# Python-for-HPC/ramba

Measured on NVIDIA H100. Metric: fused-elementwise GB/s (fp64 sin/cos/mul/add chain), higher is better.
Workload: dtype f64

## Files before the change

### ramba_b200/csrc/rb200_lean.cuh

```cuda
#pragma once
#include <cuda_runtime.h>
#include <stdint.h>

#include "rb200_vm.cuh"

namespace rb200 {

constexpr int LV = 8;

enum LeanKind { L_ACC = 0, L_REG = 1, L_SCAL = 2, L_STAGED = 3, L_DIRECT = 4, L_NONE = 7 };
enum LeanOp {
  LO_MOV = 0, LO_ADD, LO_SUB, LO_RSUB, LO_MUL, LO_DIV, LO_NEG, LO_ABS, LO_SQUARE, LO_MIN, LO_MAX,
  LO_MULADD, LO_MULSUB, LO_MULRSUB, LO_CVT, LO_RED, LO_CHAIN, LO_NUM
};

struct LInsn {
  unsigned char handler;
  unsigned char a_kind, b_kind, c_kind;
  unsigned char a_arg, b_arg, c_arg;
  unsigned char st_reg;
  unsigned char st_view;
  unsigned char red_op;
  unsigned char pad[2];
};

enum LeanChainOp { LC_ADD = 0, LC_SUB = 1, LC_RSUB = 2, LC_MUL = 3 };
struct LChainStep {
  unsigned char op, staged, pad[2];
};

struct LDirect {
  char* base;
  long long s0, s1, s2;
  int dtype;
  int pad;
};

template <class F> struct LAcc;
template <> struct LAcc<double> {
  static __device__ __forceinline__ double get(unsigned lo, unsigned hi) { return __hiloint2double((int)hi, (int)lo); }
  static __device__ __forceinline__ void put(double v, unsigned& lo, unsigned& hi) {
    lo = (unsigned)__double2loint(v);
    hi = (unsigned)__double2hiint(v);
  }
};
template <> struct LAcc<float> {
  static __device__ __forceinline__ float get(unsigned lo, unsigned) { return __uint_as_float(lo); }
  static __device__ __forceinline__ void put(float v, unsigned& lo, unsigned&) { lo = __float_as_uint(v); }
};

template <class F> __device__ __forceinline__ F lean_lds(unsigned addr);
template <> __device__ __forceinline__ double lean_lds<double>(unsigned addr) { return __longlong_as_double((long long)lds64(addr)); }
template <> __device__ __forceinline__ float lean_lds<float>(unsigned addr) { return __uint_as_float(lds32(addr)); }
template <class F> __device__ __forceinline__ void lean_sts(unsigned addr, F v);
template <> __device__ __forceinline__ void lean_sts<double>(unsigned addr, double v) { sts64(addr, (u64)__double_as_longlong(v)); }
template <> __device__ __forceinline__ void lean_sts<float>(unsigned addr, float v) {
  asm volatile("st.shared.u32 [%0], %1;" ::"r"(addr), "r"(__float_as_uint(v)) : "memory");
}

template <class F> struct LOther;
template <> struct LOther<double> { typedef float type; };
template <> struct LOther<float> { typedef double type; };

template <class F> __device__ __forceinline__ F l_add(F a, F b);
template <> __device__ __forceinline__ double l_add<double>(double a, double b) { return __dadd_rn(a, b); }
template <> __device__ __forceinline__ float l_add<float>(float a, float b) { return __fadd_rn(a, b); }
template <class F> __device__ __forceinline__ F l_sub(F a, F b);
template <> __device__ __forceinline__ double l_sub<double>(double a, double b) { return __dsub_rn(a, b); }
template <> __device__ __forceinline__ float l_sub<float>(float a, float b) { return __fsub_rn(a, b); }
template <class F> __device__ __forceinline__ F l_mul(F a, F b);
template <> __device__ __forceinline__ double l_mul<double>(double a, double b) { return __dmul_rn(a, b); }
template <> __device__ __forceinline__ float l_mul<float>(float a, float b) { return __fmul_rn(a, b); }
template <class F> __device__ __forceinline__ F l_div(F a, F b);
template <> __device__ __forceinline__ double l_div<double>(double a, double b) { return __ddiv_rn(a, b); }
template <> __device__ __forceinline__ float l_div<float>(float a, float b) { return __fdiv_rn(a, b); }

template <int LOP, class F, bool AACC, class CX> __device__ __forceinline__ void lean_exec(CX& cx, const LInsn& I) {
  F r[LV];
  if constexpr (LOP == LO_CVT) {
    typedef typename LOther<F>::type S;
    S s[LV];
    if constexpr (AACC) {
#pragma unroll
      for (int k = 0; k < LV; ++k) s[k] = LAcc<S>::get(cx.alo[k], cx.ahi[k]);
    } else {
      cx.template fetch<S>(I.a_kind, I.a_arg, s);
    }
#pragma unroll
    for (int k = 0; k < LV; ++k) r[k] = (F)s[k];
  } else {
    F a[LV];
    if constexpr (AACC) {
#pragma unroll
      for (int k = 0; k < LV; ++k) a[k] = LAcc<F>::get(cx.alo[k], cx.ahi[k]);
    } else {
      cx.template fetch<F>(I.a_kind, I.a_arg, a);
    }
    if constexpr (LOP == LO_MOV) {
#pragma unroll
      for (int k = 0; k < LV; ++k) r[k] = a[k];
    } else if constexpr (LOP == LO_CHAIN) {
#pragma unroll
      for (int k = 0; k < LV; ++k) r[k] = a[k];
#pragma unroll 1
      for (int s = 0; s < (int)I.c_arg; ++s) {
        F b[LV];
        const int cop = cx.template chain_fetch<F>((int)I.b_arg + s, b);
        if (cop == LC_ADD) {
#pragma unroll
          for (int k = 0; k < LV; ++k) r[k] = l_add<F>(r[k], b[k]);
        } else if (cop == LC_SUB) {
#pragma unroll
          for (int k = 0; k < LV; ++k) r[k] = l_sub<F>(r[k], b[k]);
        } else if (cop == LC_RSUB) {
#pragma unroll
          for (int k = 0; k < LV; ++k) r[k] = l_sub<F>(b[k], r[k]);
        } else {
#pragma unroll
          for (int k = 0; k < LV; ++k) r[k] = l_mul<F>(r[k], b[k]);
        }
      }
    } else if constexpr (LOP == LO_NEG) {
#pragma unroll
      for (int k = 0; k < LV; ++k) r[k] = -a[k];
    } else if constexpr (LOP == LO_ABS) {
#pragma unroll
      for (int k = 0; k < LV; ++k) r[k] = (F)fabs(a[k]);
    } else if constexpr (LOP == LO_SQUARE) {
#pragma unroll
      for (int k = 0; k < LV; ++k) r[k] = l_mul<F>(a[k], a[k]);
    } else if constexpr (LOP == LO_RED) {
      cx.template reduce<F>(I.b_arg, I.red_op, a);
      return;
    } else {
      F b[LV];
      cx.template fetch<F>(I.b_kind, I.b_arg, b);
      if constexpr (LOP == LO_ADD) {
#pragma unroll
        for (int k = 0; k < LV; ++k) r[k] = l_add<F>(a[k], b[k]);
      } else if constexpr (LOP == LO_SUB) {
#pragma unroll
        for (int k = 0; k < LV; ++k) r[k] = l_sub<F>(a[k], b[k]);
      } else if constexpr (LOP == LO_RSUB) {
#pragma unroll
        for (int k = 0; k < LV; ++k) r[k] = l_sub<F>(b[k], a[k]);
      } else if constexpr (LOP == LO_MUL) {
#pragma unroll
        for (int k = 0; k < LV; ++k) r[k] = l_mul<F>(a[k], b[k]);
      } else if constexpr (LOP == LO_DIV) {
#pragma unroll
        for (int k = 0; k < LV; ++k) r[k] = l_div<F>(a[k], b[k]);
      } else if constexpr (LOP == LO_MIN) {
#pragma unroll
        for (int k = 0; k < LV; ++k) r[k] = (b[k] < a[k]) ? b[k] : a[k];
      } else if constexpr (LOP == LO_MAX) {
#pragma unroll
        for (int k = 0; k < LV; ++k) r[k] = (b[k] > a[k]) ? b[k] : a[k];
      } else {
        F c[LV];
        cx.template fetch<F>(I.c_kind, I.c_arg, c);
#pragma unroll
        for (int k = 0; k < LV; ++k) {
          const F p = l_mul<F>(b[k], c[k]);
          r[k] = LOP == LO_MULADD ? l_add<F>(a[k], p) : LOP == LO_MULSUB ? l_sub<F>(a[k], p) : l_sub<F>(p, a[k]);
        }
      }
    }
  }
  if constexpr (LOP != LO_RED) {
#pragma unroll
    for (int k = 0; k < LV; ++k) LAcc<F>::put(r[k], cx.alo[k], cx.ahi[k]);
    if (I.st_reg != RB200_NOSTORE) cx.template store_reg<F>(I.st_reg, r);
    if (I.st_view != RB200_NOSTORE) cx.template store_view<F>(I.st_view, r);
  }
}

#define RB200_LEAN_CASE(LOP)                                             \
  case (LOP) * 4 + 0: lean_exec<LOP, double, false>(cx, I); break;       \
  case (LOP) * 4 + 1: lean_exec<LOP, double, true>(cx, I); break;        \
  case (LOP) * 4 + 2: lean_exec<LOP, float, false>(cx, I); break;        \
  case (LOP) * 4 + 3: lean_exec<LOP, float, true>(cx, I); break;

template <class CX> __device__ __forceinline__ void lean_dispatch(CX& cx, const LInsn& I) {
  switch (I.handler) {
    RB200_LEAN_CASE(LO_MOV)
    RB200_LEAN_CASE(LO_ADD)
    RB200_LEAN_CASE(LO_SUB)
    RB200_LEAN_CASE(LO_RSUB)
    RB200_LEAN_CASE(LO_MUL)
    RB200_LEAN_CASE(LO_DIV)
    RB200_LEAN_CASE(LO_NEG)
    RB200_LEAN_CASE(LO_ABS)
    RB200_LEAN_CASE(LO_SQUARE)
    RB200_LEAN_CASE(LO_MIN)
    RB200_LEAN_CASE(LO_MAX)
    RB200_LEAN_CASE(LO_MULADD)
    RB200_LEAN_CASE(LO_MULSUB)
    RB200_LEAN_CASE(LO_MULRSUB)
    RB200_LEAN_CASE(LO_CVT)
    RB200_LEAN_CASE(LO_RED)
    RB200_LEAN_CASE(LO_CHAIN)
    default: break;
  }
}

}
```

### ramba_b200/csrc/rb200_lean_plan.h

```cpp
#pragma once
#include <string.h>

#include "rb200_lean.cuh"

namespace rb200 {

static inline int lean_opcode(const rb200_fused_op* op, const rb200_insn& I) {
  switch (I.op) {
    case RB200_OP_MOV: return LO_MOV;
    case RB200_OP_ADD: return LO_ADD;
    case RB200_OP_SUB: return LO_SUB;
    case RB200_OP_MUL: return LO_MUL;
    case RB200_OP_DIV: return LO_DIV;
    case RB200_OP_NEG: return LO_NEG;
    case RB200_OP_ABS: return LO_ABS;
    case RB200_OP_SQUARE: return LO_SQUARE;
    case RB200_OP_MIN: return LO_MIN;
    case RB200_OP_MAX: return LO_MAX;
    case RB200_OP_MULADD: return LO_MULADD;
    case RB200_OP_MULSUB: return LO_MULSUB;
    case RB200_OP_MULRSUB: return LO_MULRSUB;
    case RB200_OP_RED: return LO_RED;
    case RB200_OP_POWI:
      if (I.b_kind == RB200_K_SCAL && (long long)op->scalars[I.b_idx] == 2) return LO_SQUARE;
      return -1;
    case RB200_OP_CVT: {
      const int src = (int)(I.imm & 0xff);
      if ((I.imm >> 8) != 0) return -1;
      if (!(src == RB200_T_F64 || src == RB200_T_F32) || src == (int)I.ctype) return -1;
      return LO_CVT;
    }
    default: return -1;
  }
}

static inline bool lean_eligible(const rb200_fused_op* op, bool allow_red) {
  if (op->n_insns < 1) return false;
  for (int i = 0; i < op->n_views; ++i)
    if (op->views[i].dtype != RB200_F32 && op->views[i].dtype != RB200_F64) return false;
  for (int i = 0; i < op->n_insns; ++i) {
    const rb200_insn& I = op->insns[i];
    if (I.ctype != RB200_T_F64 && I.ctype != RB200_T_F32) return false;
    if (I.mask_reg != RB200_NOSTORE) return false;
    const int lop = lean_opcode(op, I);
    if (lop < 0) return false;
    if (lop == LO_RED && (!allow_red || I.ctype != RB200_T_F64)) return false;
    const uint8_t kinds[3] = {I.a_kind, I.b_kind, I.c_kind};
    for (int q = 0; q < 3; ++q) {
      if (lop == LO_RED && q == 1) continue;
      if (kinds[q] == RB200_K_IOTA) return false;
    }
    if (I.a_kind == RB200_K_NONE) return false;
  }
  return true;
}

static inline void lean_translate(const rb200_fused_op* op, const int* view_kind, const int* view_arg, const int* store_arg, LInsn* out) {
  for (int i = 0; i < op->n_insns; ++i) {
    const rb200_insn& I = op->insns[i];
    LInsn L;
    memset(&L, 0, sizeof(L));
    int lop = lean_opcode(op, I);
    uint8_t kinds[3] = {I.a_kind, I.b_kind, I.c_kind};
    uint8_t idxs[3] = {I.a_idx, I.b_idx, I.c_idx};
    if (lop == LO_SQUARE || lop == LO_RED) kinds[1] = RB200_K_NONE;
    if ((lop == LO_ADD || lop == LO_MUL) && kinds[0] != RB200_K_ACC && kinds[1] == RB200_K_ACC) {
      kinds[1] = kinds[0]; idxs[1] = idxs[0];
      kinds[0] = RB200_K_ACC; idxs[0] = 0;
    } else if (lop == LO_SUB && kinds[0] != RB200_K_ACC && kinds[1] == RB200_K_ACC) {
      lop = LO_RSUB;
      kinds[1] = kinds[0]; idxs[1] = idxs[0];
      kinds[0] = RB200_K_ACC; idxs[0] = 0;
    }
    unsigned char lk[3], la[3];
    for (int q = 0; q < 3; ++q) {
      switch (kinds[q]) {
        case RB200_K_ACC: lk[q] = L_ACC; la[q] = 0; break;
        case RB200_K_REG: lk[q] = L_REG; la[q] = idxs[q]; break;
        case RB200_K_SCAL: lk[q] = L_SCAL; la[q] = idxs[q]; break;
        case RB200_K_VIEW: lk[q] = (unsigned char)view_kind[idxs[q]]; la[q] = (unsigned char)view_arg[idxs[q]]; break;
        default: lk[q] = L_NONE; la[q] = 0;
      }
    }
    L.a_kind = lk[0]; L.a_arg = la[0];
    L.b_kind = lk[1]; L.b_arg = la[1];
    L.c_kind = lk[2]; L.c_arg = la[2];
    if (lop == LO_RED) {
      L.b_arg = I.b_idx;
      L.red_op = (unsigned char)I.imm;
    }
    L.st_reg = I.st_reg;
    L.st_view = I.st_view == RB200_NOSTORE ? (unsigned char)RB200_NOSTORE : (unsigned char)store_arg[I.st_view];
    L.handler = (unsigned char)(lop * 4 + (I.ctype == RB200_T_F32 ? 2 : 0) + (L.a_kind == L_ACC ? 1 : 0));
    out[i] = L;
  }
}

static inline int lean_fuse_chains(LInsn* insns, int n, LChainStep* chain, int max_chain, int* n_chain_out) {
  int out = 0, nc = 0;
  int i = 0;
  auto chain_op = [](const LInsn& L) -> int {
    const int lop = L.handler >> 2;
    return lop == LO_ADD ? LC_ADD : lop == LO_SUB ? LC_SUB : lop == LO_RSUB ? LC_RSUB : lop == LO_MUL ? LC_MUL : -1;
  };
  while (i < n) {
    const LInsn first = insns[i];
    int j = i;
    if (chain_op(first) >= 0 && first.b_kind == L_STAGED) {
      const int cls = (first.handler >> 1) & 1;
      j = i + 1;
      while (j < n && insns[j - 1].st_reg == RB200_NOSTORE && insns[j - 1].st_view == RB200_NOSTORE && chain_op(insns[j]) >= 0 &&
             insns[j].b_kind == L_STAGED && insns[j].a_kind == L_ACC && ((insns[j].handler >> 1) & 1) == cls && nc + (j - i) + 1 <= max_chain && (j - i) < 200)
        ++j;
      if (j - i >= 2) {
        LInsn L = first;
        L.handler = (unsigned char)(LO_CHAIN * 4 + cls * 2 + (first.a_kind == L_ACC ? 1 : 0));
        L.b_kind = L_NONE;
        L.b_arg = (unsigned char)nc;
        L.c_arg = (unsigned char)(j - i);
        L.st_reg = insns[j - 1].st_reg;
        L.st_view = insns[j - 1].st_view;
        for (int q = i; q < j; ++q) {
          chain[nc].op = (unsigned char)chain_op(insns[q]);
          chain[nc].staged = insns[q].b_arg;
          ++nc;
        }
        insns[out++] = L;
        i = j;
        continue;
      }
    }
    insns[out++] = first;
    ++i;
  }
  *n_chain_out = nc;
  return out;
}

}
```

### ramba_b200/csrc/rb200_stream.cu

```cuda
#include <cuda_runtime.h>
#include <stdio.h>
#include <string.h>

#include <string>

#include "rb200_launch.h"
#include "rb200_lean.cuh"
#include "rb200_lean_plan.h"
#include "rb200_terms.h"
#include "rb200_mapred.h"
#include "rb200_stream.h"

namespace rb200 {

struct StreamCtx {
  const StreamParams& P;
  unsigned stage_s;
  unsigned reg_s;
  unsigned tid;
  bool staged_ok;
  long long row, e0;
  unsigned valid;
  unsigned alo[LV], ahi[LV];
  double racc[RB200_MAX_REDS];
// ... 74 lines not shown
  template <class F> __device__ __forceinline__ void reduce(int slot, int rop, const F (&a)[LV]) {
    if constexpr (sizeof(F) == 8) {
      if (P.mode == 1) {
#pragma unroll
        for (int k = 0; k < LV; ++k) cacc[k] = red_combine<double>(rop, cacc[k], a[k]);
        return;
      }
      double x[LV];
      const double ident = CT<double>::get(red_identity_bits(rop, RB200_T_F64));
#pragma unroll
      for (int k = 0; k < LV; ++k) x[k] = ((valid >> k) & 1u) ? (double)a[k] : ident;
#pragma unroll
      for (int w = LV / 2; w > 0; w >>= 1) {
#pragma unroll
        for (int k = 0; k < w; ++k) x[k] = red_combine<double>(rop, x[k], x[k + w]);
      }
#pragma unroll
      for (int s = 0; s < RB200_MAX_REDS; ++s)
        if (s == slot) racc[s] = red_combine<double>(rop, racc[s], x[0]);
    }
  }
};

__device__ __forceinline__ void stream_finish_reductions(const StreamParams& P, const double (&racc)[RB200_MAX_REDS]) {
  if (P.n_reds > 0) {
    __shared__ u64 wpart[RB200_MAX_REDS][kThreads / 32];
    __shared__ bool is_last;
    const int lane = threadIdx.x & 31, warp = threadIdx.x >> 5;
    for (int s = 0; s < P.n_reds; ++s) {
      const int op = P.reds[s].op;
      double mine = 0.0;
#pragma unroll
      for (int q = 0; q < RB200_MAX_REDS; ++q)
        if (q == s) mine = racc[q];
      u64 v = CT<double>::bits(mine);
#pragma unroll
      for (int o = 16; o > 0; o >>= 1) v = red_combine_bits(op, RB200_T_F64, v, __shfl_down_sync(0xffffffffu, v, o));
      if (lane == 0) wpart[s][warp] = v;
    }
    __syncthreads();
    if (threadIdx.x == 0) {
      for (int s = 0; s < P.n_reds; ++s) {
        const int op = P.reds[s].op;
        u64 v = wpart[s][0];
        for (int q = 1; q < kThreads / 32; ++q) v = red_combine_bits(op, RB200_T_F64, v, wpart[s][q]);
        P.red_partials[(long long)s * gridDim.x + blockIdx.x] = v;
      }
      __threadfence();
      const unsigned prev = atomicAdd(P.red_counter, 1u);
      is_last = (prev == gridDim.x - 1);
    }
    __syncthreads();
    if (is_last) {
      __threadfence();
      for (int s = 0; s < P.n_reds; ++s) {
        const int op = P.reds[s].op;
        u64 v = red_identity_bits(op, RB200_T_F64);
        for (unsigned b = threadIdx.x; b < gridDim.x; b += kThreads)
          v = red_combine_bits(op, RB200_T_F64, v, __ldcg(&P.red_partials[(long long)s * gridDim.x + b]));
#pragma unroll
        for (int o = 16; o > 0; o >>= 1) v = red_combine_bits(op, RB200_T_F64, v, __shfl_down_sync(0xffffffffu, v, o));
        __syncthreads();
        if (lane == 0) wpart[s][warp] = v;
        __syncthreads();
        if (threadIdx.x == 0) {
          v = wpart[s][0];
          for (int q = 1; q < kThreads / 32; ++q) v = red_combine_bits(op, RB200_T_F64, v, wpart[s][q]);
          const double vd = CT<double>::get(v);
          void* out = P.reds[s].out;
          if (P.reds[s].out_dtype == RB200_F64) {
            double* o = (double*)out;
            *o = red_combine<double>(op, *o, vd);
          } else {
            float* o = (float*)out;
            *o = (float)red_combine<double>(op, (double)*o, vd);
          }
        }
      }
      if (threadIdx.x == 0) *P.red_counter = 0u;
    }
  }
}

__global__ void __launch_bounds__(kThreads, 2) stream_kernel(const __grid_constant__ StreamParams P) {
  extern __shared__ __align__(128) unsigned char smem_raw[];
  const unsigned smem_s = (unsigned)__cvta_generic_to_shared(smem_raw);
  const unsigned tid = threadIdx.x;
  const unsigned ring_bytes = (unsigned)P.depth * P.stage_bytes;
  const unsigned regs_s = smem_s + ring_bytes;
  const unsigned mbar_s = regs_s + (unsigned)(P.n_regs + P.n_hoist) * (LV * kThreads * 8);
  if (P.n_staged > 0 && tid == 0) {
    for (int s = 0; s < P.depth; ++s) mbar_init(mbar_s + 8u * s, 1u);
    asm volatile("fence.mbarrier_init.release.cluster;" ::: "memory");
  }
  __syncthreads();

  StreamCtx cx(P);
  cx.tid = tid;
  cx.reg_s = regs_s + tid * 8u;
#pragma unroll
  for (int s = 0; s < RB200_MAX_REDS; ++s) cx.racc[s] = 0.0;
  for (int s = 0; s < P.n_reds; ++s) {
    const double ident = CT<double>::get(red_identity_bits(P.reds[s].op, RB200_T_F64));
#pragma unroll
    for (int q = 0; q < RB200_MAX_REDS; ++q)
      if (q == s) cx.racc[q] = ident;
  }

  long long n_it, base0, step_it;
  long long split = 0, col0 = 0, r0 = 0;
  if (P.mode == 0) {
    n_it = (P.n_tiles - (long long)blockIdx.x + gridDim.x - 1) / gridDim.x;
    base0 = (long long)blockIdx.x * kStreamTile;
    step_it = (long long)gridDim.x * kStreamTile;
    cx.row = 0;
  } else {
    split = blockIdx.x / (unsigned)P.n_chunks;
    const long long chunk = blockIdx.x - split * P.n_chunks;
    col0 = chunk * kStreamTile;
    r0 = split * P.rows_per_split;
    long long r1 = r0 + P.rows_per_split;
    if (r1 > P.R) r1 = P.R;
    n_it = r1 > r0 ? r1 - r0 : 0;
    base0 = r0 * P.C + col0;
    step_it = P.C;
    const double ident = CT<double>::get(red_identity_bits(P.reds[0].op, RB200_T_F64));
#pragma unroll
    for (int k = 0; k < LV; ++k) cx.cacc[k] = ident;
    cx.e0 = col0 + tid;
    cx.valid = (1u << LV) - 1u;
    cx.row = 0;
    cx.staged_ok = false;
    for (int h = 0; h < P.n_hoist; ++h) {
      if (P.hoist[h].is_f32_class) {
        float v[LV];
        cx.fetch_direct<float>(P.hoist[h].direct, v);
        cx.store_reg<float>(P.hoist[h].reg, v);
      } else {
        double v[LV];
        cx.fetch_direct<double>(P.hoist[h].direct, v);
        cx.store_reg<double>(P.hoist[h].reg, v);
      }
    }
  }

  auto tile_full = [&](long long it) -> bool { return P.mode == 1 || base0 + it * step_it + kStreamTile <= P.total; };
  auto issue = [&](long long it) {
    if (tid != 0) return;
    const unsigned slot = (unsigned)(it % P.depth);
    const unsigned bar = mbar_s + 8u * slot;
    const unsigned dst = smem_s + slot * P.stage_bytes;
    const long long eoff = base0 + it * step_it;
    unsigned bytes = 0;
    for (int j = 0; j < P.n_staged; ++j) bytes += (unsigned)(kStreamTile * P.staged[j].es);
    mbar_expect_tx(bar, bytes);
    for (int j = 0; j < P.n_staged; ++j)
      bulk_g2s(dst + P.staged[j].off, P.staged[j].base + eoff * P.staged[j].es, (unsigned)(kStreamTile * P.staged[j].es), bar);
  };

  if (P.n_staged > 0) {
    for (long long it = 0; it < P.depth - 1 && it < n_it; ++it)
      if (tile_full(it)) issue(it);
  }
  for (long long it = 0; it < n_it; ++it) {
    const bool full = tile_full(it);
    if (P.n_staged > 0) {
      __syncthreads();
      const long long nx = it + P.depth - 1;
      if (nx < n_it && tile_full(nx)) issue(nx);
      if (full) mbar_wait(mbar_s + 8u * (unsigned)(it % P.depth), (unsigned)((it / P.depth) & 1));
    }
    cx.staged_ok = full && P.n_staged > 0;
    cx.stage_s = smem_s + (unsigned)(it % (P.depth > 0 ? P.depth : 1)) * P.stage_bytes;
    if (P.mode == 0) {
      const long long e = base0 + it * step_it + tid;
      cx.e0 = e;
      unsigned valid = (1u << LV) - 1u;
      if (!full) {
        valid = 0;
#pragma unroll
        for (int k = 0; k < LV; ++k)
          if (e + (long long)k * kThreads < P.total) valid |= 1u << k;
      }
      cx.valid = valid;
    } else {
      cx.row = r0 + it;
    }
#pragma unroll 1
    for (int pc = 0; pc < P.n_insns; ++pc) {
      const LInsn I = P.insns[pc];
      lean_dispatch(cx, I);
    }
  }

  if (P.mode == 1) {
#pragma unroll
    for (int k = 0; k < LV; ++k) P.red_partials[split * P.C + col0 + tid + (long long)k * kThreads] = CT<double>::bits(cx.cacc[k]);
    return;
  }
  stream_finish_reductions(P, cx.racc);
}


template <int TV> struct STermCtx {
  unsigned stage_s, hoist_s, tid;
  bool staged_ok;
  long long row, e0;
  unsigned valid;
};

__device__ __forceinline__ void ip_add(double& a, double b) { asm("add.rn.f64 %0, %0, %1;" : "+d"(a) : "d"(b)); }
__device__ __forceinline__ void ip_sub(double& a, double b) { asm("sub.rn.f64 %0, %0, %1;" : "+d"(a) : "d"(b)); }
__device__ __forceinline__ void ip_rsub(double& a, double b) { asm("sub.rn.f64 %0, %1, %0;" : "+d"(a) : "d"(b)); }
__device__ __forceinline__ void ip_mul(double& a, double b) { asm("mul.rn.f64 %0, %0, %1;" : "+d"(a) : "d"(b)); }
__device__ __forceinline__ void ip_add(float& a, float b) { asm("add.rn.f32 %0, %0, %1;" : "+f"(a) : "f"(b)); }
__device__ __forceinline__ void ip_sub(float& a, float b) { asm("sub.rn.f32 %0, %0, %1;" : "+f"(a) : "f"(b)); }
__device__ __forceinline__ void ip_rsub(float& a, float b) { asm("sub.rn.f32 %0, %1, %0;" : "+f"(a) : "f"(b)); }
__device__ __forceinline__ void ip_mul(float& a, float b) { asm("mul.rn.f32 %0, %0, %1;" : "+f"(a) : "f"(b)); }

template <int TV, class F>
__device__ __forceinline__ void sterm_fetch(const StreamParams& P, const STermCtx<TV>& cx, const TermStep t, F (&x)[TV]) {
  int dview = t.xidx;
  if (t.xkind == X_STAGED) {
    const StreamStaged& sv = P.staged[t.xidx];
    if (cx.staged_ok) {
      if (sv.es == 4) {
        const unsigned addr = cx.stage_s + sv.off + cx.tid * 4u;
#pragma unroll
        for (int k = 0; k < TV; ++k) x[k] = (F)lean_lds<float>(addr + k * kThreads * 4);
      } else {
        const unsigned addr = cx.stage_s + sv.off + cx.tid * 8u;
#pragma unroll
        for (int k = 0; k < TV; ++k) x[k] = (F)lean_lds<double>(addr + k * kThreads * 8);
      }
      return;
    }
    dview = sv.dview;
  } else if (t.xkind == X_HOIST) {
    const unsigned base = cx.hoist_s + (unsigned)t.xidx * (TV * kThreads * 8);
    if (P.direct[P.thoist_direct[t.xidx]].dtype == RB200_F32) {
#pragma unroll
      for (int k = 0; k < TV; ++k) x[k] = (F)lean_lds<float>(base + cx.tid * 4u + k * kThreads * 4);
    } else {
#pragma unroll
      for (int k = 0; k < TV; ++k) x[k] = (F)lean_lds<double>(base + cx.tid * 8u + k * kThreads * 8);
    }
    return;
  }
  const LDirect& v = P.direct[dview];
  const long long off = cx.row * v.s1 + cx.e0 * v.s2;
  const long long step = (long long)kThreads * v.s2;
  if (v.dtype == RB200_F32) {
    const float* p = reinterpret_cast<const float*>(v.base) + off;
#pragma unroll
    for (int k = 0; k < TV; ++k, p += step) x[k] = ((cx.valid >> k) & 1u) ? (F)ldg<float>(p) : F(0);
  } else {
    const double* p = reinterpret_cast<const double*>(v.base) + off;
#pragma unroll
    for (int k = 0; k < TV; ++k, p += step) x[k] = ((cx.valid >> k) & 1u) ? (F)ldg<double>(p) : F(0);
  }
}

template <int TV, class F> __device__ __forceinline__ void sterm_store(const StreamParams& P, const STermCtx<TV>& cx, int dview, const F (&acc)[TV]) {
  const LDirect& v = P.direct[dview];
  const bool full = cx.valid == (TV == 32 ? 0xffffffffu : (1u << TV) - 1u);
  if (v.dtype == RB200_F32) {
    char* p = v.base + (cx.row * v.s1 + cx.e0 * v.s2) * 4;
    const long long step = (long long)kThreads * v.s2 * 4;
    if (full) {
#pragma unroll
      for (int k = 0; k < TV; ++k, p += step) stg<float>(reinterpret_cast<float*>(p), (float)acc[k]);
    } else {
#pragma unroll
      for (int k = 0; k < TV; ++k, p += step)
// ... 217 lines not shown
  __syncthreads();

  auto tile_full = [&](long long it) -> bool { return P.mode == 1 || base0 + it * step_it + TILE <= P.total; };
  auto issue = [&](long long it, int slot) {
    if (tid != 0) return;
    const unsigned bar = mbar_s + 8u * (unsigned)slot;
    const unsigned dst = smem_s + (unsigned)slot * P.stage_bytes;
    const long long eoff = base0 + it * step_it;
    mbar_expect_tx(bar, P.stage_bytes);
    for (int j = 0; j < P.n_staged; ++j)
      bulk_g2s(dst + P.staged[j].off, P.staged[j].base + eoff * P.staged[j].es, (unsigned)(TILE * P.staged[j].es), bar);
  };
  int islot = 0;
  if (P.n_staged > 0) {
    for (long long it = 0; it < P.depth - 1 && it < n_it; ++it) {
      if (tile_full(it)) issue(it, islot);
      islot = islot + 1 >= P.depth ? 0 : islot + 1;
    }
  }
  int slot = 0;
  unsigned par = 0;
  for (long long it = 0; it < n_it; ++it) {
    const bool full = tile_full(it);
    if (P.n_staged > 0) {
      __syncthreads();
      const long long nx = it + P.depth - 1;
      if (nx < n_it) {
        if (tile_full(nx)) issue(nx, islot);
        islot = islot + 1 >= P.depth ? 0 : islot + 1;
      }
      if (full) {
        mbar_wait(mbar_s + 8u * (unsigned)slot, (par >> slot) & 1u);
        par ^= 1u << slot;
      }
    }
    cx.staged_ok = full && P.n_staged > 0;
    cx.stage_s = smem_s + (unsigned)slot * P.stage_bytes;
    slot = slot + 1 >= P.depth ? 0 : slot + 1;
    if (P.mode == 0) {
      const long long e = base0 + it * step_it + tid;
      cx.e0 = e;
      unsigned valid = TV == 32 ? 0xffffffffu : (1u << TV) - 1u;
      if (!full) {
        valid = 0;
#pragma unroll
        for (int k = 0; k < TV; ++k)
          if (e + (long long)k * kThreads < P.total) valid |= 1u << k;
      }
      cx.valid = valid;
    } else {
      cx.row = r0 + it;
    }
    if (P.n32 > 0) {
      float a32[TV];
      sterm_steps<TV, float>(P, cx, 0, P.n32, a32, cacc, racc);
      if (P.n_terms > P.n32) {
        double a64[TV];
#pragma unroll
        for (int k = 0; k < TV; ++k) a64[k] = (double)a32[k];
        sterm_steps<TV, double>(P, cx, P.n32, P.n_terms, a64, cacc, racc);
      }
    } else {
      double a64[TV];
      sterm_steps<TV, double>(P, cx, 0, P.n_terms, a64, cacc, racc);
    }
  }

  if (P.mode == 1) {
#pragma unroll
    for (int k = 0; k < TV; ++k) P.red_partials[split * P.C + col0 + tid + (long long)k * kThreads] = CT<double>::bits(cacc[k]);
    return;
  }
  stream_finish_reductions(P, racc);
}


static bool stream_translate(const rb200_fused_op* op, StreamParams& P, bool column_mode, long long row_len) {
  bool rd[RB200_MAX_VIEWS] = {false};
  for (int i = 0; i < op->n_insns; ++i) {
    const rb200_insn& I = op->insns[i];
    const int lop = lean_opcode(op, I);
    if (I.a_kind == RB200_K_VIEW) rd[I.a_idx] = true;
    if (I.b_kind == RB200_K_VIEW && lop != LO_RED && lop != LO_SQUARE) rd[I.b_idx] = true;
    if (I.c_kind == RB200_K_VIEW) rd[I.c_idx] = true;
  }
  int view_kind[RB200_MAX_VIEWS], view_arg[RB200_MAX_VIEWS], store_arg[RB200_MAX_VIEWS];
  unsigned off = 0;
  for (int v = 0; v < op->n_views; ++v) {
    const rb200_view& vw = op->views[v];
    const int es = vw.dtype == RB200_F64 ? 8 : 4;
    LDirect& d = P.direct[P.n_direct];
    d.base = (char*)vw.base;
    d.s0 = 0;
    d.s1 = column_mode ? vw.stride[0] : 0;
    d.s2 = column_mode ? vw.stride[1] : vw.stride[0];
    d.dtype = vw.dtype;
    view_kind[v] = L_DIRECT;
    view_arg[v] = store_arg[v] = P.n_direct;
    const bool contiguous = d.s2 == 1 && (!column_mode || d.s1 == row_len);
    const bool aligned = (((uintptr_t)vw.base) & 15u) == 0 && (!column_mode || (row_len * es) % 16 == 0);
    if (rd[v] && contiguous && aligned && P.n_staged < kStreamMaxStaged) {
      StreamStaged& s = P.staged[P.n_staged];
      s.base = (const char*)vw.base;
      s.es = es;
      s.dview = P.n_direct;
      s.off = off;
      off += (unsigned)(kStreamTile * es);
      view_kind[v] = L_STAGED;
      view_arg[v] = P.n_staged;
      ++P.n_staged;
    }
    ++P.n_direct;
  }
  P.stage_bytes = off;
  P.n_insns = op->n_insns;
  P.n_regs = op->n_regs;
  lean_translate(op, view_kind, view_arg, store_arg, P.insns);
  for (int i = 0; i < op->n_scalars; ++i) P.scal[i] = op->scalars[i];
  return true;
}

static void stream_hoist_lean(StreamParams& P) {
    for (int dv = 0; dv < P.n_direct && P.n_hoist < kStreamMaxStaged; ++dv) {
      if (P.direct[dv].s1 != 0 || P.direct[dv].s2 != 1) continue;
      int cls = -1;
      bool same = true, used = false;
      for (int i = 0; i < P.n_insns; ++i) {
        const LInsn& L = P.insns[i];
        const int lop = L.handler >> 2;
        int fcls = (L.handler >> 1) & 1;
        if (lop == LO_CVT) fcls = 1 - fcls;
        const bool uses = (L.a_kind == L_DIRECT && L.a_arg == dv) || (L.b_kind == L_DIRECT && L.b_arg == dv) || (L.c_kind == L_DIRECT && L.c_arg == dv);
        if (!uses) continue;
        used = true;
        if (cls < 0) cls = fcls;
        else if (cls != fcls) same = false;
      }
      if (!used || !same) continue;
      const int reg = P.n_regs + P.n_hoist;
      if (reg >= 255) break;
      P.hoist[P.n_hoist].direct = dv;
      P.hoist[P.n_hoist].reg = reg;
      P.hoist[P.n_hoist].is_f32_class = cls;
      ++P.n_hoist;
      for (int i = 0; i < P.n_insns; ++i) {
        LInsn& L = P.insns[i];
        if (L.a_kind == L_DIRECT && L.a_arg == dv) { L.a_kind = L_REG; L.a_arg = (unsigned char)reg; }
        if (L.b_kind == L_DIRECT && L.b_arg == dv) { L.b_kind = L_REG; L.b_arg = (unsigned char)reg; }
        if (L.c_kind == L_DIRECT && L.c_arg == dv) { L.c_kind = L_REG; L.c_arg = (unsigned char)reg; }
      }
    }
  }

static void stream_layout(StreamParams& P) {
  unsigned off = 0;
  for (int j = 0; j < P.n_staged; ++j) {
    P.staged[j].off = off;
    off += (unsigned)(P.tv * kThreads * P.staged[j].es);
  }
  P.stage_bytes = off;
}

static size_t stream_smem(StreamParams& P) {
  const size_t tile = (size_t)P.tv * kThreads;
  const size_t regs = P.n_terms > 0 ? (size_t)P.n_thoist * tile * 8 : (size_t)(P.n_regs + P.n_hoist) * LV * kThreads * 8;
  const size_t budget = P.n_terms > 0 ? 70 * 1024 : 100 * 1024;
  if (regs + 1024 > budget) return 0;
  int depth = 0;
  if (P.n_staged > 0) {
    depth = (int)((budget - regs - 256) / P.stage_bytes);
    if (depth > 8) depth = 8;
    if (depth < 2) return 0;
  }
  P.depth = depth;
  return (size_t)depth * P.stage_bytes + regs + (size_t)(depth > 0 ? depth : 1) * 8 + 16;
}

bool plan_stream(const rb200_fused_op* op, int sms, int max_red_blocks, int n_split, bool use_terms, bool use_mapred, StreamPlan& T) {
  StreamParams& P = T.P;
  memset(&T, 0, sizeof(T));
  const bool column = op->n_axis_red_dims != 0;
  if (!column) {
    if (op->ndim != 1) return false;
    if (!lean_eligible(op, true)) return false;
    for (int s = 0; s < op->n_reds; ++s) {
      if (op->reds[s].ctype != RB200_T_F64) return false;
      if (op->reds[s].out_dtype != RB200_F64 && op->reds[s].out_dtype != RB200_F32) return false;
    }
    P.mode = 0;
    P.total = op->itershape[0];
  } else {
    if (op->ndim != 2 || op->n_axis_red_dims != 1 || op->n_reds != 1) return false;
    if (!lean_eligible(op, true)) return false;
    if (op->reds[0].ctype != RB200_T_F64) return false;
    const long long R = op->itershape[0], C = op->itershape[1];
    if (C % (LV * kThreads) != 0 || R < 2) return false;
    for (int i = 0; i < op->n_insns; ++i)
      if (op->insns[i].st_view != RB200_NOSTORE) return false;
    for (int v = 0; v < op->n_views; ++v) {
      const rb200_view& vw = op->views[v];
      if (vw.stride[1] != 1 || !(vw.stride[0] == C || vw.stride[0] == 0)) return false;
    }
    P.mode = 1;
    P.R = R;
    P.C = C;
    P.total = R * C;
  }
  P.tv = LV;
  stream_translate(op, P, column, P.C);
  TermBuild tb;
  tb.n_regs = P.n_regs;
  tb.direct = P.direct;
  tb.stream = true;
  tb.staged_fill = [](void*, int, int, TermStep*) -> bool { return true; };
  tb.ctx = nullptr;
  int out_view = -1;
  if (use_terms && build_terms(tb, P.insns, P.n_insns, P.terms, kMaxTerms, &P.n_terms, &P.n32, &out_view)) {
    auto src_of = [](void* ctx, const TermStep& t) -> MrSource {
      const StreamParams* Q = (const StreamParams*)ctx;
      MrSource r = {nullptr, 0, false};
      const LDirect* d = nullptr;
      if (t.xkind == X_STAGED) d = &Q->direct[Q->staged[t.xidx].dview];
      else if (t.xkind == X_DIRECT) d = &Q->direct[t.xidx];
      if (!d || d->s2 != 1) return r;
      if (Q->mode == 1 && !(d->s1 == Q->C || d->s1 == 0)) return r;
      r.base = d->base;
      r.f32 = d->dtype == RB200_F32;
      r.row_broadcast = Q->mode == 1 && d->s1 == 0;
      return r;
    };
    if (use_mapred && op->n_reds == 1 && mapred_try(P.mode, P.terms, P.n_terms, P.n32, P.scal, src_of, &P, &T.mr) == 0) {
      MrParams& M = T.mr;
      const int vec = M.src_f32 ? 4 : 2;
      bool ok = true;
      if (!column) {
        M.total = P.total;
        M.red.op = op->reds[0].op;
        M.red.ctype = op->reds[0].ctype;
        M.red.out = op->reds[0].out;
        M.red.out_dtype = op->reds[0].out_dtype;
        M.red_counter = (unsigned int*)op->red_scratch;
        M.red_partials = (u64*)((char*)op->red_scratch + 256);
        long long blocks = (P.total / (vec * 4) + kThreads - 1) / kThreads;
        long long cap = (long long)sms * 8;
        if (cap > max_red_blocks) cap = max_red_blocks;
        if (blocks > cap) blocks = cap;
        if (blocks < 1) blocks = 1;
        T.blocks = blocks;
      } else {
        const long long chunk = (long long)kThreads * vec;
        if (P.C % chunk != 0 || (P.C * (M.src_f32 ? 4 : 8)) % 16 != 0) ok = false;
        if (ok) {
          M.R = P.R;
          M.C = P.C;
          M.n_chunks = (int)(P.C / chunk);
          int eff = (int)(((long long)sms * 8) / M.n_chunks);
          if (n_split > 0 && eff > n_split) eff = n_split;
          if ((long long)eff > P.R) eff = (int)P.R;
          if (eff < 1) eff = 1;
          M.n_split = eff;
          M.rows_per_split = (P.R + eff - 1) / eff;
          M.red_partials = (u64*)op->red_scratch;
          T.eff = eff;
          T.blocks = (long long)eff * M.n_chunks;
        }
      }
      if (ok) {
        T.use_mr = true;
        T.smem = 0;
        return true;
      }
    }
    stream_layout(P);
    if (column) {
      for (int i = 0; i < P.n_terms; ++i) {
        TermStep& t = P.terms[i];
        if (t.xkind != X_DIRECT || P.direct[t.xidx].s1 != 0 || P.direct[t.xidx].s2 != 1) continue;
        int h = -1;
        for (int q = 0; q < P.n_thoist; ++q)
          if (P.thoist_direct[q] == t.xidx) h = q;
        if (h < 0 && P.n_thoist < kStreamMaxStaged) {
          h = P.n_thoist++;
          P.thoist_direct[h] = t.xidx;
        }
        if (h >= 0) {
          t.xkind = X_HOIST;
          t.xidx = (unsigned char)h;
        }
      }
    }
  } else {
    P.n_terms = 0;
    if (column) stream_hoist_lean(P);
  }
  T.smem = stream_smem(P);
  if (T.smem == 0) return false;
  const long long tile = (long long)P.tv * kThreads;
  P.n_reds = op->n_reds;
  for (int s = 0; s < op->n_reds; ++s) {
    P.reds[s].op = op->reds[s].op;
    P.reds[s].ctype = op->reds[s].ctype;
    P.reds[s].out = op->reds[s].out;
    P.reds[s].out_dtype = op->reds[s].out_dtype;
  }
  if (!column) {
    P.n_tiles = (P.total + tile - 1) / tile;
    if (op->n_reds > 0) {
      P.red_counter = (unsigned int*)op->red_scratch;
      P.red_partials = (u64*)((char*)op->red_scratch + 256);
    }
    long long blocks = P.n_tiles;
    long long cap = (long long)sms * ((P.n_terms > 0 && T.smem <= 72 * 1024) ? RB200_STREAM_MINB8 : 2);
    if (op->n_reds > 0 && cap > max_red_blocks) cap = max_red_blocks;
    if (blocks > cap) blocks = cap;
    T.blocks = blocks;
  } else {
    P.n_chunks = (int)(P.C / tile);
    const int per_sm = (P.n_terms > 0 && T.smem <= 72 * 1024) ? RB200_STREAM_MINB8 : 2;
    if (P.n_chunks > sms * per_sm) return false;
    int eff = (int)(((long long)sms * per_sm) / P.n_chunks);
    if (n_split > 0 && eff > n_split) eff = n_split;
    if ((long long)eff > P.R) eff = (int)P.R;
    if (eff < 1) eff = 1;
    P.n_split = eff;
    P.rows_per_split = (P.R + eff - 1) / eff;
    P.red_partials = (u64*)op->red_scratch;
    T.eff = eff;
    T.blocks = (long long)eff * P.n_chunks;
  }
  return true;
}

std::string describe_stream(const StreamPlan& T) {
  const StreamParams& P = T.P;
  char buf[320];
  if (T.use_mr) {
    snprintf(buf, sizeof(buf), "kernel=mapred mode=%s source=%s ops=%d(f32:%d) broadcast_operand=%d reduction=%d loads=128bit ctas=%lld", P.mode == 0 ? "global" : "columns",
             T.mr.src_f32 ? "f32" : "f64", T.mr.n32 + T.mr.n64, T.mr.n32, T.mr.vsrc ? 1 : 0, T.mr.redop, T.blocks);
    return buf;
  }
  snprintf(buf, sizeof(buf),
           "kernel=%s mode=%s staged_views=%d ring_depth=%d stage_bytes=%u direct_views=%d hoisted=%d lean_insns=%d terms=%d(f32:%d) tile=%d reds=%d "
           "ctas=%lld smem=%zu",
           P.n_terms > 0 ? "stream_terms" : "stream", P.mode == 0 ? "elementwise" : "columns", P.n_staged, P.depth, P.stage_bytes, P.n_direct,
           P.n_terms > 0 ? P.n_thoist : P.n_hoist, P.n_insns, P.n_terms, P.n32, P.tv * kThreads, P.n_reds, T.blocks, T.smem);
  return buf;
}

cudaError_t launch_stream(const StreamPlan& T, cudaStream_t stream) {
  if (T.use_mr) return mapred_launch(T.mr, (unsigned)T.blocks, stream);
  static const bool attrs = []() {
    cudaFuncSetAttribute(stream_kernel, cudaFuncAttributeMaxDynamicSharedMemorySize, 101 * 1024);
    cudaFuncSetAttribute(stream_terms_kernel<8>, cudaFuncAttributeMaxDynamicSharedMemorySize, 101 * 1024);
    return true;
  }();
  (void)attrs;
  if (T.P.n_terms > 0) stream_terms_kernel<8><<<(unsigned)T.blocks, kThreads, T.smem, stream>>>(T.P);
  else stream_kernel<<<(unsigned)T.blocks, kThreads, T.smem, stream>>>(T.P);
  return cudaGetLastError();
}

}
```

### ramba_b200/csrc/rb200_stream.h

```cpp
#pragma once
#include <cuda_runtime.h>

#include <string>

#include "rb200_lean.cuh"
#include "rb200_mapred.h"
#include "rb200_terms.h"

namespace rb200 {

constexpr int kStreamMaxStaged = 4;
constexpr int kStreamTile = LV * kThreads;

struct StreamStaged {
  const char* base;
  int es;
  int dview;
  unsigned off;
  int pad;
};

struct StreamHoist {
  int direct, reg, is_f32_class;
};

struct StreamParams {
  int mode;
  long long total, n_tiles;
  long long R, C, rows_per_split;
  int n_chunks, n_split;
  int n_staged, depth;
  unsigned stage_bytes;
  StreamStaged staged[kStreamMaxStaged];
  int n_direct;
  LDirect direct[RB200_MAX_VIEWS];
  int n_hoist;
  StreamHoist hoist[kStreamMaxStaged];
  int n_insns, n_regs;
  LInsn insns[RB200_MAX_INSNS];
  u64 scal[RB200_MAX_SCALARS];
  int n_reds;
  KRed reds[RB200_MAX_REDS];
  u64* red_partials;
  unsigned int* red_counter;
  int tv, n_terms, n32;
  int n_thoist;
  int thoist_direct[kStreamMaxStaged];
  TermStep terms[kMaxTerms];
};
constexpr int X_HOIST = 3;

struct StreamPlan {
  StreamParams P;
  size_t smem;
  long long blocks;
  int eff;
  bool use_mr;
  MrParams mr;
};

bool plan_stream(const rb200_fused_op* op, int sms, int max_red_blocks, int n_split, bool use_terms, bool use_mapred, StreamPlan& T);
std::string describe_stream(const StreamPlan& T);
cudaError_t launch_stream(const StreamPlan& T, cudaStream_t stream);

}
```

### ramba_b200/csrc/rb200_tile.cu

```cuda
#include <cuda.h>
#include <cuda_runtime.h>
#include <stdio.h>
#include <string.h>

#include <string>

#include "rb200_launch.h"
#include "rb200_lean.cuh"
#include "rb200_lean_plan.h"
#include "rb200_terms.h"
#include "rb200_tile.h"

namespace rb200 {

__device__ __forceinline__ void tma_load_3d(unsigned sdst, const CUtensorMap* tmap, int c0, int c1, int c2, unsigned mbar) {
  asm volatile(
      "cp.async.bulk.tensor.3d.shared::cluster.global.mbarrier::complete_tx::bytes [%0], [%1, {%3, %4, %5}], [%2];" ::"r"(sdst),
      "l"(tmap), "r"(mbar), "r"(c0), "r"(c1), "r"(c2)
      : "memory");
}
__device__ __forceinline__ void cp_async_mbar_arrive(unsigned mbar) {
  asm volatile("cp.async.mbarrier.arrive.noinc.shared::cta.b64 [%0];" ::"r"(mbar) : "memory");
}

// ... 411 lines not shown
          if (sl >= D) sl -= D;
        }
        mbar_wait(mbar_s + 8u * (unsigned)sl, (par >> sl) & 1u);
        par ^= 1u << sl;
        if (my_dzl >= 0) {
          int q = cur + my_dzl;
          if (q >= D) q -= D;
          asm volatile("st.shared.u32 [%0], %1;" ::"r"(table_s + ((unsigned)z & 1u) * (kTileMaxTerms * 4u) + 4u * tid),
                       "r"(smem_s + (unsigned)q * P.plane_bytes + my_off)
                       : "memory");
        }
        __syncthreads();
        if (z + P.prefetch < ze) {
          tile_request<TE>(P, &tmap, smem_s, mbar_s, (unsigned)rq, x0, y0, z + hz + P.prefetch, tid);
          rq = rq + 1 == D ? 0 : rq + 1;
        }
        cur = cur + 1 == D ? 0 : cur + 1;
      }
      cx.z = z;
      cx.table_s = table_s + ((unsigned)z & 1u) * (kTileMaxTerms * 4u);
      if (P.n32 > 0) {
        if constexpr (sizeof(TE) == 4) {
          constexpr unsigned kstep = (unsigned)(kTileRY * kTilePX * sizeof(TE));
          float a32[TV];
          term_steps<TE, TV, float>(P, cx, 0, P.n32, a32);
          if (P.fast_tail) {
            const TermStep t = P.terms[P.n32];
            const double w = __longlong_as_double((long long)P.scal[t.sidx]);
            const unsigned addr = lds32(cx.table_s + 4u * (unsigned)P.n32) + cx.tb0;
            double r[TV];
            if (t.flags & TF_NEGP) {
#pragma unroll
              for (int k = 0; k < TV; ++k) r[k] = __dsub_rn((double)a32[k], __dmul_rn((double)lean_lds<TE>(addr + k * kstep), w));
            } else if (t.flags & TF_NEGACC) {
#pragma unroll
              for (int k = 0; k < TV; ++k) r[k] = __dsub_rn(__dmul_rn((double)lean_lds<TE>(addr + k * kstep), w), (double)a32[k]);
            } else {
#pragma unroll
              for (int k = 0; k < TV; ++k) r[k] = __dadd_rn((double)a32[k], __dmul_rn((double)lean_lds<TE>(addr + k * kstep), w));
            }
            term_store<TV, double>(optr, ostep, ov.dtype, cx.valid, r);
          } else if (P.n_terms > P.n32) {
            double a64[TV];
#pragma unroll
            for (int k = 0; k < TV; ++k) a64[k] = (double)a32[k];
            term_steps<TE, TV, double>(P, cx, P.n32, P.n_terms, a64);
            term_store<TV, double>(optr, ostep, ov.dtype, cx.valid, a64);
          } else {
            term_store<TV, float>(optr, ostep, ov.dtype, cx.valid, a32);
          }
        }
      } else {
        double a64[TV];
        term_steps<TE, TV, double>(P, cx, 0, P.n_terms, a64);
        term_store<TV, double>(optr, ostep, ov.dtype, cx.valid, a64);
      }
      optr += oplane;
    }
  }
}

typedef CUresult (*EncodeTiledFn)(CUtensorMap*, CUtensorMapDataType, cuuint32_t, void*, const cuuint64_t*, const cuuint64_t*, const cuuint32_t*,
                                  const cuuint32_t*, CUtensorMapInterleave, CUtensorMapSwizzle, CUtensorMapL2promotion, CUtensorMapFloatOOBfill);

static EncodeTiledFn encode_tiled_fn() {
  static const EncodeTiledFn fn = []() -> EncodeTiledFn {
    void* p = nullptr;
    cudaDriverEntryPointQueryResult q;
    if (cudaGetDriverEntryPoint("cuTensorMapEncodeTiled", &p, cudaEnableDefault, &q) == cudaSuccess && q == cudaDriverEntryPointSuccess) return (EncodeTiledFn)p;
    return nullptr;
  }();
  return fn;
}

static long long floor_div(long long a, long long b) {
  long long q = a / b;
  if ((a % b != 0) && (a < 0)) --q;
  return q;
}

bool plan_stencil_tile(const rb200_fused_op* op, int sms, bool use_terms, bool use_tma, TilePlan& T) {
  if (op->ndim != 2 && op->ndim != 3) return false;
  if (op->n_reds != 0 || op->n_axis_red_dims != 0) return false;
  if (!lean_eligible(op, false)) return false;
  const int nd = op->ndim;
  TileParams& P = T.P;
  memset(&T, 0, sizeof(T));
  P.Z = nd == 3 ? op->itershape[0] : 1;
  P.Y = op->itershape[nd - 2];
  P.X = op->itershape[nd - 1];
  if (P.X >= (1ll << 31) || P.Y >= (1ll << 31) || P.Z >= (1ll << 31)) return false;

  bool rd[RB200_MAX_VIEWS] = {false}, wr[RB200_MAX_VIEWS] = {false};
  for (int i = 0; i < op->n_insns; ++i) {
    const rb200_insn& I = op->insns[i];
    const int lop = lean_opcode(op, I);
    if (I.a_kind == RB200_K_VIEW) rd[I.a_idx] = true;
    if (I.b_kind == RB200_K_VIEW && lop != LO_RED && lop != LO_SQUARE) rd[I.b_idx] = true;
    if (I.c_kind == RB200_K_VIEW) rd[I.c_idx] = true;
    if (I.st_view != RB200_NOSTORE) wr[I.st_view] = true;
  }
  auto S = [&](int v, int d) -> long long {
    if (nd == 3) return op->views[v].stride[d];
    return d == 0 ? 0 : op->views[v].stride[d - 1];
  };

  int best_ref = -1, best_n = 0;
  int member[RB200_MAX_VIEWS];
  long long mdz[RB200_MAX_VIEWS], mdy[RB200_MAX_VIEWS], mdx[RB200_MAX_VIEWS];
  for (int r = 0; r < op->n_views; ++r) {
    if (!rd[r] || wr[r] || S(r, 2) != 1 || S(r, 1) < 64 || (nd == 3 && S(r, 0) < S(r, 1))) continue;
    if (!op->views[r].alloc_lo || !op->views[r].alloc_hi) continue;
    const int es = op->views[r].dtype == RB200_F64 ? 8 : 4;
    int n = 0;
    for (int v = 0; v < op->n_views; ++v) {
      if (!rd[v] || wr[v] || op->views[v].dtype != op->views[r].dtype) continue;
      if (S(v, 0) != S(r, 0) || S(v, 1) != S(r, 1) || S(v, 2) != 1) continue;
      if (op->views[v].alloc_lo != op->views[r].alloc_lo) continue;
      const long long db = (const char*)op->views[v].base - (const char*)op->views[r].base;
      if (db % es != 0) continue;
      long long delta = db / es, dz = 0;
      if (nd == 3 && S(r, 0) > 0) {
        dz = floor_div(delta + S(r, 0) / 2, S(r, 0));
        delta -= dz * S(r, 0);
      }
      const long long dy = floor_div(delta + S(r, 1) / 2, S(r, 1));
      const long long dx = delta - dy * S(r, 1);
      if (dz < -3 || dz > 3 || dy < -8 || dy > 8 || dx < -8 || dx > 8) continue;
      ++n;
    }
    if (n > best_n) {
      best_n = n;
      best_ref = r;
    }
  }
  int view_kind[RB200_MAX_VIEWS], view_arg[RB200_MAX_VIEWS], store_arg[RB200_MAX_VIEWS];
  for (int v = 0; v < op->n_views; ++v) {
    view_kind[v] = L_DIRECT;
    view_arg[v] = 0;
    store_arg[v] = 0;
  }
  int es = 4;
  if (best_n >= 2) {
    const int r = best_ref;
    es = op->views[r].dtype == RB200_F64 ? 8 : 4;
    long long lo[3] = {0, 0, 0}, hi[3] = {0, 0, 0};
    int n = 0;
    for (int v = 0; v < op->n_views; ++v) {
      if (!rd[v] || wr[v] || op->views[v].dtype != op->views[r].dtype) continue;
      if (S(v, 0) != S(r, 0) || S(v, 1) != S(r, 1) || S(v, 2) != 1) continue;
      if (op->views[v].alloc_lo != op->views[r].alloc_lo) continue;
      const long long db = (const char*)op->views[v].base - (const char*)op->views[r].base;
      if (db % es != 0) continue;
      long long delta = db / es, dz = 0;
      if (nd == 3 && S(r, 0) > 0) {
        dz = floor_div(delta + S(r, 0) / 2, S(r, 0));
        delta -= dz * S(r, 0);
      }
      const long long dy = floor_div(delta + S(r, 1) / 2, S(r, 1));
      const long long dx = delta - dy * S(r, 1);
      if (dz < -3 || dz > 3 || dy < -8 || dy > 8 || dx < -8 || dx > 8) continue;
      member[n] = v;
      mdz[n] = dz; mdy[n] = dy; mdx[n] = dx;
      if (dz < lo[0]) lo[0] = dz;
      if (dz > hi[0]) hi[0] = dz;
      if (dy < lo[1]) lo[1] = dy;
      if (dy > hi[1]) hi[1] = dy;
// ... 197 lines not shown
```

Before: 2602.

## Route fp64 sin/cos/sincos chains through the lean stream kernel

```diff
diff --git a/ramba_b200/csrc/rb200_lean.cuh b/ramba_b200/csrc/rb200_lean.cuh
--- a/ramba_b200/csrc/rb200_lean.cuh
+++ b/ramba_b200/csrc/rb200_lean.cuh
@@ -11,7 +11,7 @@
 enum LeanKind { L_ACC = 0, L_REG = 1, L_SCAL = 2, L_STAGED = 3, L_DIRECT = 4, L_NONE = 7 };
 enum LeanOp {
   LO_MOV = 0, LO_ADD, LO_SUB, LO_RSUB, LO_MUL, LO_DIV, LO_NEG, LO_ABS, LO_SQUARE, LO_MIN, LO_MAX,
-  LO_MULADD, LO_MULSUB, LO_MULRSUB, LO_CVT, LO_RED, LO_CHAIN, LO_NUM
+  LO_MULADD, LO_MULSUB, LO_MULRSUB, LO_CVT, LO_RED, LO_CHAIN, LO_SINCOS, LO_NUM
 };
 
 struct LInsn {
@@ -21,7 +21,8 @@
   unsigned char st_reg;
   unsigned char st_view;
   unsigned char red_op;
-  unsigned char pad[2];
+  unsigned char st2;
+  unsigned char imm;
 };
 
 enum LeanChainOp { LC_ADD = 0, LC_SUB = 1, LC_RSUB = 2, LC_MUL = 3 };
@@ -132,6 +133,19 @@
     } else if constexpr (LOP == LO_RED) {
       cx.template reduce<F>(I.b_arg, I.red_op, a);
       return;
+    } else if constexpr (LOP == LO_SINCOS) {
+      F sn[LV], cs[LV];
+      sincos_v<LV>(a, sn, cs);
+      const bool want_cos = I.imm != 0;
+#pragma unroll
+      for (int k = 0; k < LV; ++k) r[k] = want_cos ? cs[k] : sn[k];
+      if (I.st2 != RB200_NOSTORE) {
+        F park[LV];
+#pragma unroll
+        for (int k = 0; k < LV; ++k) park[k] = want_cos ? sn[k] : cs[k];
+        cx.template store_reg<F>(I.st2, park);
+        if (I.c_arg != RB200_NOSTORE) cx.template store_view<F>(I.c_arg, park);
+      }
     } else {
       F b[LV];
       cx.template fetch<F>(I.b_kind, I.b_arg, b);
@@ -181,7 +195,7 @@
   case (LOP) * 4 + 2: lean_exec<LOP, float, false>(cx, I); break;        \
   case (LOP) * 4 + 3: lean_exec<LOP, float, true>(cx, I); break;
 
-template <class CX> __device__ __forceinline__ void lean_dispatch(CX& cx, const LInsn& I) {
+template <bool TRIG = false, class CX> __device__ __forceinline__ void lean_dispatch(CX& cx, const LInsn& I) {
   switch (I.handler) {
     RB200_LEAN_CASE(LO_MOV)
     RB200_LEAN_CASE(LO_ADD)
@@ -200,8 +214,13 @@
     RB200_LEAN_CASE(LO_CVT)
     RB200_LEAN_CASE(LO_RED)
     RB200_LEAN_CASE(LO_CHAIN)
-    default: break;
-  }
-}
-
-}
+    default:
+      if constexpr (TRIG) {
+        if (I.handler == LO_SINCOS * 4 + 0) lean_exec<LO_SINCOS, double, false>(cx, I);
+        else if (I.handler == LO_SINCOS * 4 + 1) lean_exec<LO_SINCOS, double, true>(cx, I);
+      }
+      break;
+  }
+}
+
+}
diff --git a/ramba_b200/csrc/rb200_lean_plan.h b/ramba_b200/csrc/rb200_lean_plan.h
--- a/ramba_b200/csrc/rb200_lean_plan.h
+++ b/ramba_b200/csrc/rb200_lean_plan.h
@@ -21,6 +21,9 @@
     case RB200_OP_MULSUB: return LO_MULSUB;
     case RB200_OP_MULRSUB: return LO_MULRSUB;
     case RB200_OP_RED: return LO_RED;
+    case RB200_OP_SIN:
+    case RB200_OP_COS:
+    case RB200_OP_SINCOS: return LO_SINCOS;
     case RB200_OP_POWI:
       if (I.b_kind == RB200_K_SCAL && (long long)op->scalars[I.b_idx] == 2) return LO_SQUARE;
       return -1;
@@ -34,7 +37,13 @@
   }
 }
 
-static inline bool lean_eligible(const rb200_fused_op* op, bool allow_red) {
+static inline bool lean_has_trig(const rb200_fused_op* op) {
+  for (int i = 0; i < op->n_insns; ++i)
+    if (lean_opcode(op, op->insns[i]) == LO_SINCOS) return true;
+  return false;
+}
+
+static inline bool lean_eligible(const rb200_fused_op* op, bool allow_red, bool allow_trig) {
   if (op->n_insns < 1) return false;
   for (int i = 0; i < op->n_views; ++i)
     if (op->views[i].dtype != RB200_F32 && op->views[i].dtype != RB200_F64) return false;
@@ -45,6 +54,10 @@
     const int lop = lean_opcode(op, I);
     if (lop < 0) return false;
     if (lop == LO_RED && (!allow_red || I.ctype != RB200_T_F64)) return false;
+    if (lop == LO_SINCOS) {
+      if (!allow_trig || I.ctype != RB200_T_F64 || I.b_kind != RB200_K_NONE) return false;
+      if (I.c_kind != RB200_K_NONE && !(I.op == RB200_OP_SINCOS && I.c_kind == RB200_K_VIEW)) return false;
+    }
     const uint8_t kinds[3] = {I.a_kind, I.b_kind, I.c_kind};
     for (int q = 0; q < 3; ++q) {
       if (lop == LO_RED && q == 1) continue;
@@ -64,6 +77,7 @@
     uint8_t kinds[3] = {I.a_kind, I.b_kind, I.c_kind};
     uint8_t idxs[3] = {I.a_idx, I.b_idx, I.c_idx};
     if (lop == LO_SQUARE || lop == LO_RED) kinds[1] = RB200_K_NONE;
+    if (lop == LO_SINCOS) kinds[2] = RB200_K_NONE;
     if ((lop == LO_ADD || lop == LO_MUL) && kinds[0] != RB200_K_ACC && kinds[1] == RB200_K_ACC) {
       kinds[1] = kinds[0]; idxs[1] = idxs[0];
       kinds[0] = RB200_K_ACC; idxs[0] = 0;
@@ -88,6 +102,12 @@
     if (lop == LO_RED) {
       L.b_arg = I.b_idx;
       L.red_op = (unsigned char)I.imm;
+    }
+    if (lop == LO_SINCOS) {
+      const bool pair = I.op == RB200_OP_SINCOS;
+      L.imm = (unsigned char)((I.op == RB200_OP_COS || (pair && I.imm != 0)) ? 1 : 0);
+      L.st2 = pair ? I.st2 : (unsigned char)RB200_NOSTORE;
+      L.c_arg = (unsigned char)((pair && I.c_kind == RB200_K_VIEW) ? store_arg[I.c_idx] : RB200_NOSTORE);
     }
     L.st_reg = I.st_reg;
     L.st_view = I.st_view == RB200_NOSTORE ? (unsigned char)RB200_NOSTORE : (unsigned char)store_arg[I.st_view];
diff --git a/ramba_b200/csrc/rb200_stream.cu b/ramba_b200/csrc/rb200_stream.cu
--- a/ramba_b200/csrc/rb200_stream.cu
+++ b/ramba_b200/csrc/rb200_stream.cu
@@ -180,6 +180,7 @@
   }
 }
 
+template <bool TRIG>
 __global__ void __launch_bounds__(kThreads, 2) stream_kernel(const __grid_constant__ StreamParams P) {
   extern __shared__ __align__(128) unsigned char smem_raw[];
   const unsigned smem_s = (unsigned)__cvta_generic_to_shared(smem_raw);
@@ -287,7 +288,7 @@
 #pragma unroll 1
     for (int pc = 0; pc < P.n_insns; ++pc) {
       const LInsn I = P.insns[pc];
-      lean_dispatch(cx, I);
+      lean_dispatch<TRIG>(cx, I);
     }
   }
 
@@ -671,7 +672,7 @@
     const int lop = lean_opcode(op, I);
     if (I.a_kind == RB200_K_VIEW) rd[I.a_idx] = true;
     if (I.b_kind == RB200_K_VIEW && lop != LO_RED && lop != LO_SQUARE) rd[I.b_idx] = true;
-    if (I.c_kind == RB200_K_VIEW) rd[I.c_idx] = true;
+    if (I.c_kind == RB200_K_VIEW && lop != LO_SINCOS) rd[I.c_idx] = true;
   }
   int view_kind[RB200_MAX_VIEWS], view_arg[RB200_MAX_VIEWS], store_arg[RB200_MAX_VIEWS];
   unsigned off = 0;
@@ -771,7 +772,7 @@
   const bool column = op->n_axis_red_dims != 0;
   if (!column) {
     if (op->ndim != 1) return false;
-    if (!lean_eligible(op, true)) return false;
+    if (!lean_eligible(op, true, true)) return false;
     for (int s = 0; s < op->n_reds; ++s) {
       if (op->reds[s].ctype != RB200_T_F64) return false;
       if (op->reds[s].out_dtype != RB200_F64 && op->reds[s].out_dtype != RB200_F32) return false;
@@ -780,7 +781,7 @@
     P.total = op->itershape[0];
   } else {
     if (op->ndim != 2 || op->n_axis_red_dims != 1 || op->n_reds != 1) return false;
-    if (!lean_eligible(op, true)) return false;
+    if (!lean_eligible(op, true, false)) return false;
     if (op->reds[0].ctype != RB200_T_F64) return false;
     const long long R = op->itershape[0], C = op->itershape[1];
     if (C % (LV * kThreads) != 0 || R < 2) return false;
@@ -797,6 +798,13 @@
   }
   P.tv = LV;
   stream_translate(op, P, column, P.C);
+  T.trig = lean_has_trig(op);
+  if (T.trig) {
+    for (int i = 0; i < P.n_insns; ++i) {
+      const LInsn& L = P.insns[i];
+      if (L.a_kind == L_DIRECT || L.b_kind == L_DIRECT || L.c_kind == L_DIRECT) return false;
+    }
+  }
   TermBuild tb;
   tb.n_regs = P.n_regs;
   tb.direct = P.direct;
@@ -930,22 +938,24 @@
   }
   snprintf(buf, sizeof(buf),
            "kernel=%s mode=%s staged_views=%d ring_depth=%d stage_bytes=%u direct_views=%d hoisted=%d lean_insns=%d terms=%d(f32:%d) tile=%d reds=%d "
-           "ctas=%lld smem=%zu",
+           "ctas=%lld smem=%zu trig=%d",
            P.n_terms > 0 ? "stream_terms" : "stream", P.mode == 0 ? "elementwise" : "columns", P.n_staged, P.depth, P.stage_bytes, P.n_direct,
-           P.n_terms > 0 ? P.n_thoist : P.n_hoist, P.n_insns, P.n_terms, P.n32, P.tv * kThreads, P.n_reds, T.blocks, T.smem);
+           P.n_terms > 0 ? P.n_thoist : P.n_hoist, P.n_insns, P.n_terms, P.n32, P.tv * kThreads, P.n_reds, T.blocks, T.smem, T.trig ? 1 : 0);
   return buf;
 }
 
 cudaError_t launch_stream(const StreamPlan& T, cudaStream_t stream) {
   if (T.use_mr) return mapred_launch(T.mr, (unsigned)T.blocks, stream);
   static const bool attrs = []() {
-    cudaFuncSetAttribute(stream_kernel, cudaFuncAttributeMaxDynamicSharedMemorySize, 101 * 1024);
+    cudaFuncSetAttribute(stream_kernel<false>, cudaFuncAttributeMaxDynamicSharedMemorySize, 101 * 1024);
+    cudaFuncSetAttribute(stream_kernel<true>, cudaFuncAttributeMaxDynamicSharedMemorySize, 101 * 1024);
     cudaFuncSetAttribute(stream_terms_kernel<8>, cudaFuncAttributeMaxDynamicSharedMemorySize, 101 * 1024);
     return true;
   }();
   (void)attrs;
   if (T.P.n_terms > 0) stream_terms_kernel<8><<<(unsigned)T.blocks, kThreads, T.smem, stream>>>(T.P);
-  else stream_kernel<<<(unsigned)T.blocks, kThreads, T.smem, stream>>>(T.P);
+  else if (T.trig) stream_kernel<true><<<(unsigned)T.blocks, kThreads, T.smem, stream>>>(T.P);
+  else stream_kernel<false><<<(unsigned)T.blocks, kThreads, T.smem, stream>>>(T.P);
   return cudaGetLastError();
 }
 
diff --git a/ramba_b200/csrc/rb200_stream.h b/ramba_b200/csrc/rb200_stream.h
--- a/ramba_b200/csrc/rb200_stream.h
+++ b/ramba_b200/csrc/rb200_stream.h
@@ -56,6 +56,7 @@
   long long blocks;
   int eff;
   bool use_mr;
+  bool trig;
   MrParams mr;
 };
 
diff --git a/ramba_b200/csrc/rb200_tile.cu b/ramba_b200/csrc/rb200_tile.cu
--- a/ramba_b200/csrc/rb200_tile.cu
+++ b/ramba_b200/csrc/rb200_tile.cu
@@ -517,7 +517,7 @@
 bool plan_stencil_tile(const rb200_fused_op* op, int sms, bool use_terms, bool use_tma, TilePlan& T) {
   if (op->ndim != 2 && op->ndim != 3) return false;
   if (op->n_reds != 0 || op->n_axis_red_dims != 0) return false;
-  if (!lean_eligible(op, false)) return false;
+  if (!lean_eligible(op, false, false)) return false;
   const int nd = op->ndim;
   TileParams& P = T.P;
   memset(&T, 0, sizeof(T));
```

Result: no change. 2608 (median of 6 runs) (+0.3%).
